# strukturag/libheif

Measured on AMD Instinct MI355X. Metric: Mpixels/s HEIC 4:2:0 8-bit decode, higher is better.
Workload: dtype u8; 1 GPU; 2048 x 3840x2160 HEIC 4:2:0 8-bit stills per GPU and step, WPP, CTB 64, fused YCbCr->RGB24; stage_overlap=False, distinct_contents=256, parallelism=replicas x1

## Files before the change

### libheif_amd/csrc/parse_bins_lds_gfx950.h

```cpp
#define PC_LDS_HEAD_Q   "v_lshrrev_b32 %[vt], 10, %[R]\n\tv_and_b32 %[vt], 24, %[vt]\n\t"
#define PC_LDS_LPS                                                                                                                 \
  "ds_read_b32 %[vn], %[vr] offset:%c[tnext]\n\t"                                                                                   \
  "v_sub_u32 %[val], %[val], %[R]\n\t"                                                                                              \
  "v_ffbh_u32 %[vt], %[vl]\n\t"                                                                                                     \
  "v_add_u32 %[vt], -16, %[vt]\n\t"                                                                                                 \
  "v_lshlrev_b32 %[R], %[vt], %[vl]\n\t"                                                                                            \
  "v_add_u32 %[vt], -7, %[vt]\n\t"                                                                                                  \
  "v_lshlrev_b32 %[val], %[vt], %[val]\n\t"                                                                                         \
  "v_add_u32 %[bits], %[vt], %[bits]\n\t"                                                                                           \
  "v_and_b32 %[vt], 0x10000, %[vst]\n\t"                                                                                            \
  "v_xor_b32 %[vb], 1, %[vb]\n\t"                                                                                                   \
  "s_waitcnt lgkmcnt(0)\n\t"                                                                                                        \
  "v_xor_b32 %[vn], %[vn], %[vt]\n\t"
#if HIPDEC_PARSE_LDS_WIN
#define PC_LDS_REFILL(SLOW)                                                                                                        \
  "s_cmp_lt_u32 %[pos], %[flim]\n\t"                                                                                                \
  "s_cbranch_scc0 " SLOW "\n\t"                                                                                                     \
  "v_lshl_add_u32 %[val], %[vbyte], %[bits], %[val]\n\t"                                                                            \
  "v_add_u32 %[vpos], 1, %[vpos]\n\t"                                                                                               \
  "s_add_u32 %[pos], %[pos], 1\n\t"                                                                                                 \
  "ds_read_u8 %[vbyte], %[vpos] offset:%c[wwin]\n\t"                                                                                \
  "v_add_u32 %[bits], -8, %[bits]\n\t"
#define PC_LDS_WIN_WAIT "s_waitcnt lgkmcnt(0)\n\t"
#define PC_LDS_WIN_STATE(s) [vbyte] "+v"((s).vbyte), [vpos] "+v"((s).vpos),
// ... 26 lines not shown
  PC_LDS_EXP                                                                                                                        \
  "v_and_b32 %[vr], 0xfc, %[vst]\n\t"                                                                                               \
  "ds_read_b32 %[vrow], %[vr] offset:%c[tlps]\n\t"                                                                                  \
  "v_lshrrev_b32 %[vb], 16, %[vst]\n\t"                                                                                             \
  "v_pk_sub_u16 %[vn], %[vst], 4 clamp\n\t"                                                                                         \
  "s_waitcnt lgkmcnt(0)\n\t"                                                                                                        \
  "v_bfe_u32 %[vl], %[vrow], %[vt], 8\n\t"                                                                                          \
  "v_mad_i32_i24 %[R], %[vl], %[m128], %[R]\n\t"                                                                                    \
  "v_cmp_lt_u32_e32 vcc, %[val], %[R]\n\t"                                                                                          \
  "s_cbranch_vccz " LPS_LABEL "\n\t"                                                                                                \
  "v_cmp_gt_u32_e32 vcc, 0x8000, %[R]\n\t"
#define PC_LDS_MPS_SHIFT "v_lshlrev_b32 %[R], 1, %[R]\n\tv_lshlrev_b32 %[val], 1, %[val]\n\tv_add_u32 %[bits], 1, %[bits]\n"
#define PC_LDS_OFFSETS [tlps] "i"(__builtin_offsetof(Lds, tlps)), [tnext] "i"(__builtin_offsetof(Lds, tnext)), [vctx] "i"(__builtin_offsetof(Lds, vctx))
PC_DEV uint32_t pc_lds_ctx_addr(CtxGroup grp, int lane) { return (uint32_t)__builtin_offsetof(Lds, ctx) + 4u * (uint32_t)(grp.base + lane); }

PC_DEV int decode_bin(PS& s, CtxRef grp, int ctx_lane)
{
  uint32_t r, flag;
  [[maybe_unused]] uint32_t st, row;
  uint32_t vst, vrow, vt, vl, vn, vr, vb;
  const uint32_t va = pc_lds_ctx_addr(grp, ctx_lane);
  uint32_t pos = pc_uni(s.pos);
  const uint32_t flim = pc_uni(s.fast_limit);
  asm volatile(
    "ds_read_b32 %[vst], %[va]\n\t"
    "s_mov_b32 %[flag], 0\n\t"
    PC_LDS_HEAD_Q
    "s_waitcnt lgkmcnt(0)\n\t"
    PC_LDS_CORE("1f")
    "s_cbranch_vccz 6f\n\t"
    PC_LDS_MPS_SHIFT
    "s_branch 2f\n"
    "1:\n\t"
    PC_LDS_LPS
    "2:\n\t"
    "v_cmp_lt_i32_e32 vcc, -1, %[bits]\n\t"
// ... 3 lines not shown
    "s_branch 6f\n"
    "3:\n\t"
    "s_mov_b32 %[flag], 1\n"
    "6:\n\t"
    "ds_write_b32 %[va], %[vn]\n\t"
    "v_readfirstlane_b32 %[r], %[vb]\n\t"
    : [R] "+v"(s.range), [val] "+v"(s.value), [bits] "+v"(s.bits_needed), [pos] "+s"(pos), PC_LDS_WIN_STATE(s)
      [r] "=&s"(r), PC_LDS_WIN_TEMPS(st, row) [flag] "=&s"(flag),
      [vst] "=&v"(vst), [vrow] "=&v"(vrow), [vt] "=&v"(vt), [vl] "=&v"(vl), [vn] "=&v"(vn), [vr] "=&v"(vr), [vb] "=&v"(vb)
    : [va] "v"(va), PC_LDS_WIN_IN(s), [flim] "s"(flim), [m128] "v"(0xffffff80u), PC_LDS_OFFSETS
    : "vcc", "scc", "memory");
  s.pos = pc_uni(pos);
  if (__builtin_expect(pc_uni(flag) != 0u, 0)) refill_byte(s);
  return (int)pc_uni(r);
}

#define PC_LDS_SIG_ITER(P, CA, CB, NEXT)                                                                                           \
  "1" P "0:\n\t"                                                                                                                    \
  "ds_read_b32 %[vst], %[" CA "]\n\t"                                                                                               \
  "v_add_u32 %[vj], -4, %[vj]\n\t"                                                                                                  \
  "ds_read_b32 %[" CB "], %[vj] offset:%c[vctx]\n\t"                                                                                \
  PC_LDS_HEAD_Q                                                                                                                     \
  "s_waitcnt lgkmcnt(1)\n\t"                                                                                                        \
  PC_LDS_CORE("1" P "1f")                                                                                                           \
  "s_cbranch_vccnz 1" P "2f\n"                                                                                                      \
  "1" P "4:\n\t"                                                                                                                    \
  "ds_write_b32 %[" CA "], %[vn]\n\t"                                                                                               \
  "v_lshl_or_b32 %[vacc], %[vacc], 1, %[vb]\n\t"                                                                                    \
  "s_add_u32 %[j], %[j], -1\n\t"                                                                                                    \
  "s_cbranch_scc1 " NEXT "\n\t"                                                                                                     \
  "s_branch 190f\n"                                                                                                                 \
  "1" P "1:\n\t"                                                                                                                    \
  PC_LDS_LPS                                                                                                                        \
  "s_branch 1" P "3f\n"                                                                                                             \
  "1" P "2:\n\t"                                                                                                                    \
  PC_LDS_MPS_SHIFT                                                                                                                  \
  "1" P "3:\n\t"                                                                                                                    \
  "v_cmp_lt_i32_e32 vcc, -1, %[bits]\n\t"                                                                                           \
  "s_cbranch_vccz 1" P "4b\n\t"                                                                                                     \
  PC_LDS_REFILL("1" P "5f")                                                                                                         \
  "s_branch 1" P "4b\n"                                                                                                             \
  "1" P "5:\n\t"                                                                                                                    \
  "ds_write_b32 %[" CA "], %[vn]\n\t"                                                                                               \
  "v_lshl_or_b32 %[vacc], %[vacc], 1, %[vb]\n\t"                                                                                    \
  "s_add_u32 %[j], %[j], -1\n\t"                                                                                                    \
  "s_mov_b32 %[flag], 1\n\t"                                                                                                        \
  "s_branch 190f\n"

PC_DEV uint32_t decode_sig_run(PS& s, const VReg& vctx, int n_start)
{
  (void)vctx;
  uint32_t vacc = 0;
  asm volatile("v_mov_b32 %0, 0" : "=v"(vacc));
  int32_t j = __builtin_amdgcn_readfirstlane(n_start - 1);
  for (;;) {
    uint32_t flag, t;
    [[maybe_unused]] uint32_t st, row;
    uint32_t vst, vrow, vt, vl, vn, vr, vb, vca, vcb, vj;
    uint32_t pos = pc_uni(s.pos);
    const uint32_t flim = pc_uni(s.fast_limit);
    asm volatile(
      "s_lshl_b32 %[t], %[j], 2\n\t"
      "s_add_u32 %[t], %[t], 4\n\t"
      "s_mov_b32 %[flag], 0\n\t"
      "v_mov_b32 %[vj], %[t]\n\t"
      "ds_read_b32 %[vca], %[vj] offset:%c[vctx]\n\t"
      "s_waitcnt lgkmcnt(0)\n\t"
      PC_LDS_SIG_ITER("0", "vca", "vcb", "110f")
      PC_LDS_SIG_ITER("1", "vcb", "vca", "100b")
      "190:\n\t"
      PC_LDS_WIN_WAIT
      : [R] "+v"(s.range), [val] "+v"(s.value), [bits] "+v"(s.bits_needed), [pos] "+s"(pos), [j] "+s"(j), [vacc] "+v"(vacc), PC_LDS_WIN_STATE(s)
        [flag] "=&s"(flag), PC_LDS_WIN_TEMPS(st, row) [t] "=&s"(t),
        [vst] "=&v"(vst), [vrow] "=&v"(vrow), [vt] "=&v"(vt), [vl] "=&v"(vl), [vn] "=&v"(vn), [vr] "=&v"(vr), [vb] "=&v"(vb),
        [vca] "=&v"(vca), [vcb] "=&v"(vcb), [vj] "=&v"(vj)
      : PC_LDS_WIN_IN(s), [flim] "s"(flim), [m128] "v"(0xffffff80u), PC_LDS_OFFSETS
      : "vcc", "scc", "memory");
    s.pos = pc_uni(pos);
    if (__builtin_expect(__builtin_amdgcn_readfirstlane((int)flag) != 0, 0)) refill_byte(s);
    j = __builtin_amdgcn_readfirstlane(j);
    if (j < 0) break;
  }
  return pc_uni(vacc) << 1;
}

PC_DEV uint32_t decode_g1_run(PS& s, int base_lane, int n, int& g_io)
{
  uint32_t vgb = 0, vg = 0;
  int32_t m = __builtin_amdgcn_readfirstlane(n - 1);
  const uint32_t vbase = pc_lds_ctx_addr(PS::ctxC, base_lane);
  asm volatile("v_mov_b32 %0, 0\n\tv_mov_b32 %1, %2" : "=&v"(vgb), "=&v"(vg) : "s"((uint32_t)__builtin_amdgcn_readfirstlane(g_io)));
// ... 133 lines not shown
```

### libheif_amd/csrc/parse_core.h

```cpp
#pragma once
#include <stdint.h>
#include "hevc_device.h"

#if defined(HIPDEC_HOST_EMU)
#include <string.h>
#define PC_DEV static inline
inline uint64_t hipdec_emu_path_counts[8] = {};
#define PC_COUNT(k) (hipdec_emu_path_counts[k]++)
inline uint64_t hipdec_emu_glue_counts[32] = {};
#define PC_GLUE(k) (hipdec_emu_glue_counts[k]++)
struct VReg { uint32_t v[64]; };
#define PC_VEC_BEGIN for (int lane = 0; lane < 64; lane++) { (void)lane;
#define PC_VEC_END }
#define PC_L(r) ((r).v[lane])
PC_DEV uint32_t pc_rdlane(const VReg& r, int l) { return r.v[l & 63]; }
PC_DEV void pc_wrlane(VReg& r, int l, uint32_t x) { r.v[l & 63] = x; }
PC_DEV void pc_wrlane_v(VReg& r, int l, uint32_t x) { r.v[l & 63] = x; }
PC_DEV uint32_t pc_uni(uint32_t x) { return x; }
PC_DEV int pc_clz(uint32_t x) { return x ? __builtin_clz(x) : 32; }
PC_DEV int pc_ffs(uint32_t x) { return __builtin_ffs((int)x); }
PC_DEV int pc_popc(uint32_t x) { return __builtin_popcount(x); }
PC_DEV uint64_t pc_ballot(const VReg& r) { uint64_t m = 0; for (int l = 0; l < 64; l++) if (r.v[l]) m |= 1ull << l; return m; }
typedef uint32_t UReg;
PC_DEV UReg pc_vec(uint32_t x) { return x; }
// ... 40 lines not shown
#ifndef HIPDEC_PARSE_CHROMA_GENERAL
#define HIPDEC_PARSE_CHROMA_GENERAL 1
#endif
#ifndef HIPDEC_PARSE_LDS_CTX
#define HIPDEC_PARSE_LDS_CTX 0
#endif
#ifndef HIPDEC_PARSE_LDS_MAPS
#define HIPDEC_PARSE_LDS_MAPS HIPDEC_PARSE_LDS_CTX
#endif
#ifndef HIPDEC_PARSE_LDS_WIN
#define HIPDEC_PARSE_LDS_WIN HIPDEC_PARSE_LDS_CTX
#endif
#ifndef HIPDEC_PARSE_LEAN_GLUE
#define HIPDEC_PARSE_LEAN_GLUE HIPDEC_PARSE_LDS_CTX
#endif
#ifndef HIPDEC_PARSE_INTER
#define HIPDEC_PARSE_INTER 0
#endif

namespace hipdec {
namespace pcore {

struct Lds {
  alignas(16) uint32_t park[SAVE_DWORDS];
#if HIPDEC_PARSE_LDS_CTX
  alignas(16) uint32_t ctx[3 * 64];
  uint32_t tlps[64];
  uint32_t tnext[64];
  uint32_t vctx[16];
#endif
#if HIPDEC_PARSE_LDS_MAPS
  uint32_t umap[5 * 64];
#endif
#if HIPDEC_PARSE_LDS_WIN
  uint32_t wwin[128 + 2];
#endif
};
#if HIPDEC_PARSE_LDS_MAPS
struct UMap { int base; };
typedef UMap MapRef;
#define PC_MAP_SYNC() PC_LDS_SYNC()
#define PC_MAP_DW(s, m) ((s).L->umap[((m).base >> 2) + lane])
#else
typedef VReg& MapRef;
#define PC_MAP_DW(s, m) PC_L(m)
#define PC_MAP_SYNC() do { } while (0)
#endif
#if HIPDEC_PARSE_LDS_CTX
struct CtxGroup { int base; };
typedef CtxGroup CtxRef;
#else
typedef VReg& CtxRef;
// ... 32 lines not shown
  int32_t chroma_format_idc, bit_depth_luma, bit_depth_chroma, log2_min_cu_qp_delta_size;
  uint32_t tools;
  uint32_t pcm;
  int32_t slice_qp_y, deblock, sao_luma, sao_chroma;
  int32_t x_ctb, y_ctb, ctb_avail;
  int32_t is_cu_qp_delta_coded, cu_qp_delta_val, qpy_pred, last_qp_y, cur_qp_y;
  int32_t cu_tq_bypass;
  Lds* L;
#if HIPDEC_PARSE_INTER
  int32_t is_p, num_ref_idx, max_merge_cand, init_type, amp, max_th_depth_inter;
  int32_t is_b, num_ref_idx_l1, mvd_l1_zero;
  MotionSyntax* msyn;
#endif
};
enum : uint32_t { TOOL_SDH = 1, TOOL_TS = 2, TOOL_CUQPD = 4, TOOL_TQBYPASS = 8 };

PC_DEV uint32_t interleave4(uint32_t x, uint32_t y)
{
  x = (x | (x << 2)) & 0x33; x = (x | (x << 1)) & 0x55;
  y = (y | (y << 2)) & 0x33; y = (y | (y << 1)) & 0x55;
  return x | (y << 1);
}
PC_DEV uint32_t compact1by1(uint32_t v)
{
  v &= 0x55555555u; v = (v | (v >> 1)) & 0x33333333u; v = (v | (v >> 2)) & 0x0f0f0f0fu; v = (v | (v >> 4)) & 0x00ff00ffu;
  return v;
}

PC_DEV bool pc_is444(const PS& s) { return HIPDEC_PARSE_CHROMA_GENERAL && s.chroma_format_idc == 3; }
PC_DEV bool pc_is422(const PS& s) { return HIPDEC_PARSE_CHROMA_GENERAL && s.chroma_format_idc == 2; }
// ... 141 lines not shown
{
  s.pos = start; s.end = end; s.zeros = 0; s.win_base = 0xfffff000u; s.fast_limit = 0;
  s.range = pc_vec(510u << 7); s.bits_needed = pc_vec((uint32_t)-8);
  const uint32_t b0 = read_byte(s), b1 = read_byte(s);
  s.value = pc_vec((b0 << 8) | b1);
}
PC_DEV void cabac_restart(PS& s)
{
  s.range = pc_vec(510u << 7); s.bits_needed = pc_vec((uint32_t)-8);
  const uint32_t b0 = read_byte(s), b1 = read_byte(s);
  s.value = pc_vec((b0 << 8) | b1);
}
PC_DEV void refill_byte(PS& s) { s.value += read_byte_v(s) << s.bits_needed; s.bits_needed -= 8u; }

#if HIPDEC_PARSE_LDS_CTX
PC_DEV int decode_bin_cxx(PS& s, CtxRef grp, int ctx_lane)
{
  uint32_t* const cv = &s.L->ctx[grp.base + ctx_lane];
  const uint32_t st = pc_uni(*cv);
  const uint32_t row = pc_uni(s.L->tlps[(st & 0xfcu) >> 2]);
  const UReg lps = (row >> ((s.range >> 10) & 24u)) & 255u;
  UReg range = s.range - (lps << 7);
  uint32_t nst;
  int bin;
  UReg nb;
  if (__builtin_expect(pc_any(s.value < range), 1)) {
    bin = (int)(st >> 16);
    nst = st - (((st & 0xfcu) != 0u) ? 4u : 0u);
    nb = 1u - (range >> 15);
    range <<= nb;
  } else {
    bin = (int)((st >> 16) ^ 1u);
    nb = (UReg)pc_clz(lps) - 23u;
    s.value -= range;
    range = lps << (nb + 7u);
    nst = pc_uni(s.L->tnext[(st & 0xfcu) >> 2]) ^ (st & 0x10000u);
  }
  PC_VEC_BEGIN if (lane == 0) *cv = nst; PC_VEC_END
  s.range = range;
  s.value <<= nb;
  s.bits_needed += nb;
  if (__builtin_expect(pc_any((int32_t)s.bits_needed >= 0), 0)) refill_byte(s);
  return bin;
}
#else
PC_DEV int decode_bin_cxx(PS& s, VReg& grp, int ctx_lane)
{
  const uint32_t st = pc_rdlane(grp, ctx_lane);
  const uint32_t row = pc_rdlane(s.t_lps, (int)st);
  const UReg lps = (row >> ((s.range >> 10) & 24u)) & 255u;
  UReg range = s.range - (lps << 7);
  const UReg vst = pc_vec(st);
  UReg nst;
  int bin;
  UReg nb;
  if (__builtin_expect(pc_any(s.value < range), 1)) {
    bin = (int)(st >> 16);
    nst = vst - (((vst & 63u) != 0u) ? 1u : 0u);
    nb = 1u - (range >> 15);
// ... 31 lines not shown
{
  int i = 0;
  while (i < max && decode_bin(s, grp, base_lane + (i >> shift))) i++;
  return i;
}
PC_DEV uint32_t decode_g1_run(PS& s, int base_lane, int n, int& g)
{
  uint32_t gb = 0;
  for (int i = 0; i < n; i++) {
    const int b = decode_bin(s, s.ctxC, base_lane + (g > 3 ? 3 : g));
    gb = (gb << 1) | (uint32_t)b;
    if (b) g = 0; else if (g > 0) g++;
  }
  return gb;
}
PC_DEV uint32_t decode_sig_run(PS& s, const VReg& vctx, int n_start)
{
  uint32_t sig = 0;
  int k = n_start;
  do sig |= (uint32_t)decode_bin(s, s.ctxB, (int)pc_rdlane(vctx, k)) << k; while (--k > 0);
  return sig;
}
#endif

PC_DEV int decode_bypass(PS& s)
{
  s.value <<= 1;
  s.bits_needed += 1u;
  if (pc_any((int32_t)s.bits_needed >= 0)) { s.bits_needed = pc_vec((uint32_t)-8); s.value += read_byte_v(s); }
  if (pc_any(s.value >= s.range)) { s.value -= s.range; return 1; }
  return 0;
}
PC_DEV uint32_t decode_bypass_multi(PS& s, int n)
{
  s.value <<= n;
  s.bits_needed += (uint32_t)n;
// ... 71 lines not shown
    s.L->tlps[lane] = lps_row;
    s.L->tnext[lane] = (lane < 63 ? (uint32_t)(62 - c_next_lps[ps]) << 2 : 0u) | (lane == 62 ? 0x10000u : 0u);
    PC_L(s.t_next) = (uint32_t)c_diag8[lane] << 8;
#else
    PC_L(s.t_lps) = lps_row;
    PC_L(s.t_next) = (lane < 63 ? (uint32_t)(62 - c_next_lps[ps]) : 0u) | (lane == 62 ? 0x10000u : 0u) | ((uint32_t)c_diag8[lane] << 8);
#endif
  PC_VEC_END
  {
    VReg inv;
    PC_VEC_BEGIN PC_L(inv) = 0u; PC_VEC_END
    for (int k = 0; k < 64; k++) pc_wrlane(inv, (int)((pc_rdlane(s.t_next, k) >> 8) & 63u), (uint32_t)k);
    PC_VEC_BEGIN PC_L(s.t_next) |= PC_L(inv) << 24; PC_VEC_END
  }
}

PC_DEV int left_cb_log2(PS& s, int ux, int uy)
{
  if (ux > 0) return (int)(map_get(s, s.m_size, (int)interleave4((uint32_t)ux - 1, (uint32_t)uy)) >> 4);
  if (s.ctb_avail & AV_LEFT) return (int)((pc_rdlane(s.p_left, uy) & 255u) >> 4);
  return 0;
}
PC_DEV int up_cb_log2(PS& s, int ux, int uy)
{
  if (uy > 0) return (int)(map_get(s, s.m_size, (int)interleave4((uint32_t)ux, (uint32_t)uy - 1)) >> 4);
  if (s.ctb_avail & AV_UP) return (int)(((pc_rdlane(s.up, 9 + (ux >> 2)) >> ((ux & 3) * 8)) & 255u) >> 4);
  return 0;
}
PC_DEV void derive_qp_pred(PS& s, int ux, int uy)
{
// ... 115 lines not shown
  }
  PC_COUNT(2);
  if (!(s.pos < s.fast_limit)) PC_COUNT(3);
  return pc_vec((uint32_t)decode_remaining(s, (int)pc_uni(rice)));
}
PC_DEV void scan_sb(PS& s, int lg, int scan_idx, int i, int& xs, int& ys)
{
  if (lg == 0) { xs = 0; ys = 0; }
  else if (lg == 1) {
    if (scan_idx == 1) { xs = i & 1; ys = i >> 1; }
    else { xs = i >> 1; ys = i & 1; }
  } else if (lg == 2) { const uint32_t v = (uint32_t)(PC_DIAG4 >> (i * 4)) & 15u; xs = (int)(v & 3u); ys = (int)(v >> 2); }
  else { const uint32_t v = (pc_rdlane(s.t_next, i) >> 8) & 63u; xs = (int)(v & 7u); ys = (int)(v >> 3); }
}

PC_DEV int residual_coding(PS& s, int log2n, int c_idx, int pred_mode, int16_t* dst)
{
  const int n = 1 << log2n;
  int ts = 0;
  if ((s.tools & TOOL_TS) && !s.cu_tq_bypass && log2n <= 2) ts = decode_bin(s, s.ctxA, A_TRANSFORM_SKIP + (c_idx ? 1 : 0));
  int ctx_offset, ctx_shift;
  if (c_idx == 0) { ctx_offset = 3 * (log2n - 2) + ((log2n - 1) >> 2); ctx_shift = (log2n + 1) >> 2; }
  else { ctx_offset = 15; ctx_shift = log2n - 2; }
  const int c_max = (log2n << 1) - 1;
  const int px = decode_unary_ctx_run(s, s.ctxA, A_LAST_X + ctx_offset, ctx_shift, c_max);
  const int py = decode_unary_ctx_run(s, s.ctxA, A_LAST_Y + ctx_offset, ctx_shift, c_max);
  int last_x = px, last_y = py;
  if (px > 3) last_x = (1 << ((px >> 1) - 1)) * (2 + (px & 1)) + decode_bypass_bits(s, (px >> 1) - 1);
  if (py > 3) last_y = (1 << ((py >> 1) - 1)) * (2 + (py & 1)) + decode_bypass_bits(s, (py >> 1) - 1);
  int scan_idx = 0;
  if (log2n == 2 || (log2n == 3 && (c_idx == 0 || pc_is444(s)))) {
    if (pred_mode >= 6 && pred_mode <= 14) scan_idx = 2;
    else if (pred_mode >= 22 && pred_mode <= 30) scan_idx = 1;
  }
  if (scan_idx == 2) { const int t = last_x; last_x = last_y; last_y = t; }
  if (last_x >= n || last_y >= n) { s.err = DEV_ERR_SYNTAX; zero_uncoded_sub_blocks(dst, log2n, 0); return ts; }
  const uint64_t scan4 = scan_idx == 0 ? PC_DIAG4 : (scan_idx == 1 ? PC_HORZ4 : PC_VERT4);

  const int lg = log2n - 2;
  int last_sb, last_pos;
  {
    const int xs_t = last_x >> 2, ys_t = last_y >> 2;
    const uint32_t r_t = (uint32_t)((last_x & 3) | ((last_y & 3) << 2));
#if HIPDEC_PARSE_LEAN_GLUE
    last_pos = scan_idx == 0 ? (int)((uint32_t)(PC_INV_DIAG4 >> (r_t * 4u)) & 15u) : (scan_idx == 1 ? (int)r_t : (int)(((r_t & 3u) << 2) | (r_t >> 2)));
#else
    const uint64_t inv4 = scan_idx == 0 ? PC_INV_DIAG4 : (scan_idx == 1 ? PC_INV_HORZ4 : PC_INV_VERT4);
    last_pos = (int)((uint32_t)(inv4 >> (r_t * 4u)) & 15u);
#endif
    if (lg == 0) last_sb = 0;
    else if (lg == 1) last_sb = scan_idx == 1 ? (xs_t | (ys_t << 1)) : ((xs_t << 1) | ys_t);
    else if (lg == 2) last_sb = (int)((uint32_t)(PC_INV_DIAG4 >> ((uint32_t)(xs_t | (ys_t << 2)) * 4u)) & 15u);
    else last_sb = (int)((pc_rdlane(s.t_next, xs_t | (ys_t << 3)) >> 24) & 63u);
  }
  uint64_t csbf = 0;
  const int sbw = 1 << lg;
  (void)sbw;
  if (ts) PC_GLUE(0);
  PC_GLUE(c_idx ? 3 + log2n : log2n - 1);
  if (log2n <= 3) PC_GLUE((log2n == 2 ? 7 : 10) + scan_idx);
  if (lg > 0 && last_sb == 0) PC_GLUE(13);
  if (lg > 0 && last_sb == (1 << (2 * lg)) - 1) PC_GLUE(14);
  if (s.cu_tq_bypass) PC_GLUE(23);
  if (pc_is422(s)) PC_GLUE(27);
  if (pc_is444(s)) PC_GLUE(28);
#if HIPDEC_PARSE_LEAN_GLUE
  int g1_zero = 0;
  const int sdh = (s.tools & TOOL_SDH) != 0 && !s.cu_tq_bypass;
  const int sig_dc = (c_idx == 0 && log2n > 2) ? 3 : 0;
  const int sig_base = log2n == 2 ? (c_idx ? 27 : 0) : (c_idx == 0 ? 3 + (log2n == 3 ? (scan_idx == 0 ? 9 : 15) : 21) : 27 + (log2n == 3 ? 9 : 12));
#else
  int g1_carry = 1, first_sb_with_g1 = 1;
  const int sdh = (s.tools & TOOL_SDH) != 0;
#endif
  VReg vovf;
  PC_VEC_BEGIN PC_L(vovf) = 0u; PC_VEC_END
  for (int i = last_sb; i >= 0; i--) {
    int infer_dc = 0, coded;
#if HIPDEC_PARSE_LEAN_GLUE
    int pos;
    if (lg == 3) pos = (int)((pc_rdlane(s.t_next, i) >> 8) & 63u);
    else if (lg == 2) { const uint32_t v = (uint32_t)(PC_DIAG4 >> (i * 4)) & 15u; pos = (int)((v & 3u) | ((v & 12u) << 1)); }
    else if (lg == 1) pos = scan_idx == 1 ? ((i & 1) | ((i & 2) << 2)) : ((i >> 1) | ((i & 1) << 3));
    else pos = 0;
    const uint32_t nb = (uint32_t)(csbf >> pos) & ((pos & 7) == 7 ? 0x100u : 0x102u);
    if (i < last_sb && i > 0) {
      coded = decode_bin(s, s.ctxA, A_CODED_SUB_BLOCK + (nb ? 1 : 0) + (c_idx ? 2 : 0));
      infer_dc = 1;
      PC_GLUE(coded ? 17 : 16); if (nb & 2u) PC_GLUE(18); if (nb & 0x100u) PC_GLUE(19); if (!nb) PC_GLUE(20);
    } else coded = 1;
    if (!coded) continue;
    const uint32_t pat = log2n == 2 ? 0u : (nb == 0u ? PC_SIGPAT0 : (nb == 2u ? PC_SIGPAT1 : (nb == 0x100u ? PC_SIGPAT2 : PC_SIGPAT3)));
    const int sig_off = sig_base - (pos ? 0 : sig_dc);
    const int xs = pos, ys = 0;
#else
    int xs, ys;
    scan_sb(s, lg, scan_idx, i, xs, ys);
    const int right = (xs < sbw - 1) ? (int)((csbf >> (ys * 8 + xs + 1)) & 1) : 0;
    const int below = (ys < sbw - 1) ? (int)((csbf >> ((ys + 1) * 8 + xs)) & 1) : 0;
    if (i < last_sb && i > 0) {
      coded = decode_bin(s, s.ctxA, A_CODED_SUB_BLOCK + ((right | below) ? 1 : 0) + (c_idx ? 2 : 0));
      infer_dc = 1;
      PC_GLUE(coded ? 17 : 16); if (right) PC_GLUE(18); if (below) PC_GLUE(19); if (!(right | below)) PC_GLUE(20);
    } else coded = 1;
    if (!coded) continue;
    uint32_t pat;
    int sig_off;
    if (log2n == 2) { pat = 0; sig_off = c_idx ? 27 : 0; }
    else {
      const int prev_csbf = right | (below << 1);
      pat = prev_csbf == 0 ? PC_SIGPAT0 : (prev_csbf == 1 ? PC_SIGPAT1 : (prev_csbf == 2 ? PC_SIGPAT2 : PC_SIGPAT3));
      if (c_idx == 0) sig_off = ((xs | ys) ? 3 : 0) + ((log2n == 3) ? (scan_idx == 0 ? 9 : 15) : 21);
      else sig_off = 27 + ((log2n == 3) ? 9 : 12);
    }
#endif
    VReg vctx;
    {
      const int dc_sb = (xs | ys) == 0;
      PC_VEC_BEGIN
        const uint32_t r = (uint32_t)(scan4 >> ((lane & 15) * 4)) & 15u;
        uint32_t c;
        if (log2n == 2) c = (uint32_t)sig_off + (uint32_t)((PC_CTXIDXMAP4 >> (r * 4)) & 15u);
        else if (dc_sb && r == 0) c = c_idx ? 27u : 0u;
        else c = (uint32_t)sig_off + ((pat >> (r * 2)) & 3u);
        PC_L(vctx) = c;
#if HIPDEC_PARSE_LDS_CTX
        if (lane < 16) s.L->vctx[lane] = (uint32_t)__builtin_offsetof(Lds, ctx) + 4u * (uint32_t)(PS::ctxB.base + B_SIG_COEFF) + 4u * c;
#endif
      PC_VEC_END
    }
    uint32_t sig = 0;
    int n_start = 15;
    if (i == last_sb) { sig = 1u << last_pos; n_start = last_pos - 1; }
    if (n_start > 0) {
      sig |= decode_sig_run(s, vctx, n_start);
    }
    if (n_start >= 0) {
      if (infer_dc && !sig) sig = 1u;
      else sig |= (uint32_t)decode_bin(s, s.ctxB, B_SIG_COEFF + (int)pc_rdlane(vctx, 0));
    }
    if (!sig) continue;
#if HIPDEC_PARSE_LEAN_GLUE
    csbf |= 1ull << pos;
#else
    csbf |= 1ull << (ys * 8 + xs);
#endif
#if HIPDEC_PARSE_LEAN_GLUE
    const int ctx_set = ((i == 0 || c_idx > 0) ? 0 : 2) + g1_zero;
#else
    int ctx_set = (i == 0 || c_idx > 0) ? 0 : 2;
    if (!first_sb_with_g1 && g1_carry == 0) ctx_set++;
    first_sb_with_g1 = 0;
#endif
    const int last_sig_pos = 31 - pc_clz(sig), first_sig_pos = pc_ffs(sig) - 1;
// ... 855 lines not shown
  s.is_cu_qp_delta_coded = 0; s.cu_qp_delta_val = 0; s.qpy_pred = s.slice_qp_y; s.last_qp_y = s.slice_qp_y; s.cur_qp_y = s.slice_qp_y;
  s.cu_tq_bypass = 0;

  const int units_log2 = 2 * (s.log2_ctb - 2);
  const int units = 1 << units_log2;
  const int uw = 1 << (s.log2_ctb - 2);
  const int ctb_size = 1 << s.log2_ctb;
  const int n_mincb_log2 = 2 * (s.log2_ctb - s.log2_min_cb);

  load_tables(s);
  PC_VEC_BEGIN
    PC_MAP_DW(s, s.m_size) = 0; PC_MAP_DW(s, s.m_flags) = 0; PC_MAP_DW(s, s.m_ipm) = 0; PC_MAP_DW(s, s.m_ipmc) = 0; PC_MAP_DW(s, s.m_qp) = 0;
    PC_L(s.p_left) = 0; PC_L(s.up) = 0; PC_L(s.sao) = 0; PC_L(s.sao_left) = 0;
#if HIPDEC_PARSE_LDS_CTX
    for (int g = 0; g < 3; g++) s.L->ctx[g * 64 + lane] = 0;
    if (lane < 16) s.L->vctx[lane] = (uint32_t)__builtin_offsetof(Lds, ctx);
#else
    PC_L(s.ctxA) = 0; PC_L(s.ctxB) = 0; PC_L(s.ctxC) = 0;
#endif
    PC_L(s.win) = 0; PC_L(s.win_next) = 0;
  PC_VEC_END
  PC_MAP_SYNC();
  uint32_t k0 = 0;
  uint32_t* saved = A.saved + (size_t)sub_idx * SAVE_DWORDS;
  if (pool) k0 = pc_load_wt_uni(A.resume_k + sub_idx);
  if (k0 == 0) cabac_start(s, byte_start, byte_end);
  else load_row_state(s, saved, 1);

  for (uint32_t k = k0; k < num_ctbs && !s.err; k++) {
    if (pool && A.yield_ctbs && k > k0 && (k - k0) % A.yield_ctbs == 0) {
      save_row_state(s, A.resume_k + sub_idx, saved, k);
// ... 217 lines not shown
    sub = uload32(&A.waves[wave_idx].first); stride = uload32(&A.waves[wave_idx].stride);
    end = uload32(&A.waves[wave_idx].end); lag = uload32(&A.waves[wave_idx].start_lag);
  } else {
    const uint32_t n_init = A.num_waves < 64u ? A.num_waves : 64u;
    for (uint32_t s0 = wave_idx; wave_idx < n_init && s0 < A.num_subs; s0 += n_init) {
      const int32_t dep = (int32_t)uload32(&A.subs[s0].dep_sub);
      if (dep < 0) pool_push(A, s0);
      else {
        uint32_t need = 2u;
        const uint32_t dep_len = uload32(&A.subs[s0].dep_len);
        if (need > dep_len || (uload32(&A.subs[s0].wpp_sync) & 255u) == 2u) need = dep_len;
        if (pool_arm(A, s0, (uint32_t)dep, need)) pool_push(A, s0);
      }
    }
  }
#if defined(HIPDEC_POOL_TRACE) && !defined(HIPDEC_HOST_EMU)
  unsigned long long tr_start = 0, tr_last = 0, tr_idle = 0, tr_tasks = 0, tr_busy = 0, tr_now0 = wall_clock64();
#endif
  for (;;) {
    uint32_t* slot = A.queue;
#if defined(HIPDEC_POOL_TRACE) && !defined(HIPDEC_HOST_EMU)
    tr_now0 = wall_clock64();
#endif
    if (!pool) { if (sub >= end) return; }
    else {
#if defined(HIPDEC_POOL_TRACE) && !defined(HIPDEC_HOST_EMU)
      const unsigned long long tr_now = wall_clock64();
      if (tr_tasks == 0 && tr_idle == 0) tr_start = tr_now;
      if (threadIdx.x == 0 && A.trace) {
        unsigned long long* tr = A.trace + (size_t)wave_idx * 32;
// ... 48 lines not shown
```

### libheif_amd/csrc/parse_tables.h

```cpp
#pragma once
#include <stdint.h>
#ifndef PC_CONST
#define PC_CONST static const
#endif

namespace hipdec {
namespace pcore {

enum : int {
  A_SAO_MERGE = 0, A_SAO_TYPE = 1, A_SPLIT_CU = 2 , A_CU_TQ_BYPASS = 5, A_PART_MODE = 6, A_PREV_INTRA_LUMA = 7,
  A_INTRA_CHROMA = 8, A_SPLIT_TRANSFORM = 9 , A_CBF_LUMA = 12 , A_CBF_CHROMA = 14 , A_CU_QP_DELTA = 18 ,
  A_TRANSFORM_SKIP = 20 , A_LAST_X = 22 , A_LAST_Y = 40 , A_CODED_SUB_BLOCK = 58 ,
  A_CBF_CHROMA4 = 62 ,
  B_SIG_COEFF = 0, B_GREATER2 = 44,
  C_GREATER1 = 0,
  C_SKIP_FLAG = 24 , C_PRED_MODE = 27, C_PART_MODE_INTER = 28 , C_MERGE_FLAG = 31,
  C_MERGE_IDX = 32, C_REF_IDX = 33 , C_MVD_GT0 = 35, C_MVD_GT1 = 36, C_MVP_FLAG = 37, C_RQT_ROOT_CBF = 38,
  C_INTER_PRED_IDC = 39
};

PC_CONST uint8_t c_init[3][64] = {
  {153, 200, 139, 141, 157, 154, 184, 184, 63, 153, 138, 138, 111, 141, 94, 138, 182, 154, 154, 154, 139, 139,
   110, 110, 124, 125, 140, 153, 125, 127, 140, 109, 111, 143, 127, 111, 79, 108, 123, 63,
   110, 110, 124, 125, 140, 153, 125, 127, 140, 109, 111, 143, 127, 111, 79, 108, 123, 63,
// ... 71 lines not shown
  uint32_t w = 0;
  for (int r = 0; r < 16; r++) {
    const int x = r & 3, y = r >> 2;
    int v = 2;
    if (prev_csbf == 0) v = (x + y == 0) ? 2 : (x + y < 3) ? 1 : 0;
    else if (prev_csbf == 1) v = (y == 0) ? 2 : (y == 1) ? 1 : 0;
    else if (prev_csbf == 2) v = (x == 0) ? 2 : (x == 1) ? 1 : 0;
    else v = 2;
    w |= (uint32_t)v << (2 * r);
  }
  return w;
}
constexpr uint32_t PC_SIGPAT0 = pc_sigpat(0), PC_SIGPAT1 = pc_sigpat(1), PC_SIGPAT2 = pc_sigpat(2), PC_SIGPAT3 = pc_sigpat(3);
static_assert(PC_SIGPAT0 == 0x00010516u && PC_SIGPAT1 == 0x000055AAu && PC_SIGPAT2 == 0x06060606u && PC_SIGPAT3 == 0xAAAAAAAAu, "sig patterns");

}
}
```

Baseline: 19940 Mpixel/s.

## Precompute sig_coeff context-address rows and TU descriptors in LDS tables

Builds compile-time tables of per-position sig_coeff_flag context LDS addresses, grouped by TU size, component, scan and neighbour pattern, plus a per-TU-kind descriptor holding ctx offsets, scan words and sub-block scan offsets. These tables are copied into LDS at kernel start. The residual-coding sig run now reads 16-bit context addresses straight from a table row, replacing the per-sub-block vector computation of vctx and its LDS write. The aim is to cut scalar/vector glue and syncs in the hot CABAC residual path, at the cost of extra LDS footprint, a startup copy, and more complex address bookkeeping.

```diff
diff --git a/libheif_amd/csrc/parse_bins_lds_gfx950.h b/libheif_amd/csrc/parse_bins_lds_gfx950.h
--- a/libheif_amd/csrc/parse_bins_lds_gfx950.h
+++ b/libheif_amd/csrc/parse_bins_lds_gfx950.h
@@ -64,12 +64,11 @@
 #define PC_LDS_OFFSETS [tlps] "i"(__builtin_offsetof(Lds, tlps)), [tnext] "i"(__builtin_offsetof(Lds, tnext)), [vctx] "i"(__builtin_offsetof(Lds, vctx))
 PC_DEV uint32_t pc_lds_ctx_addr(CtxGroup grp, int lane) { return (uint32_t)__builtin_offsetof(Lds, ctx) + 4u * (uint32_t)(grp.base + lane); }
 
-PC_DEV int decode_bin(PS& s, CtxRef grp, int ctx_lane)
+PC_DEV int decode_bin_at(PS& s, uint32_t va)
 {
   uint32_t r, flag;
   [[maybe_unused]] uint32_t st, row;
   uint32_t vst, vrow, vt, vl, vn, vr, vb;
-  const uint32_t va = pc_lds_ctx_addr(grp, ctx_lane);
   uint32_t pos = pc_uni(s.pos);
   const uint32_t flim = pc_uni(s.fast_limit);
   asm volatile(
@@ -103,12 +102,19 @@
   if (__builtin_expect(pc_uni(flag) != 0u, 0)) refill_byte(s);
   return (int)pc_uni(r);
 }
-
+PC_DEV int decode_bin(PS& s, CtxRef grp, int ctx_lane) { return decode_bin_at(s, pc_lds_ctx_addr(grp, ctx_lane)); }
+
+#if HIPDEC_PARSE_TU_TABLES
+#define PC_LDS_SIG_ROW_IN [srow] "s"(srow),
+#define PC_LDS_SIG_NEXT(CB) "v_add_u32 %[vj], -2, %[vj]\n\tds_read_u16 %[" CB "], %[vj]\n\t"
+#else
+#define PC_LDS_SIG_ROW_IN
+#define PC_LDS_SIG_NEXT(CB) "v_add_u32 %[vj], -4, %[vj]\n\tds_read_b32 %[" CB "], %[vj] offset:%c[vctx]\n\t"
+#endif
 #define PC_LDS_SIG_ITER(P, CA, CB, NEXT)                                                                                           \
   "1" P "0:\n\t"                                                                                                                    \
   "ds_read_b32 %[vst], %[" CA "]\n\t"                                                                                               \
-  "v_add_u32 %[vj], -4, %[vj]\n\t"                                                                                                  \
-  "ds_read_b32 %[" CB "], %[vj] offset:%c[vctx]\n\t"                                                                                \
+  PC_LDS_SIG_NEXT(CB)                                                                                                               \
   PC_LDS_HEAD_Q                                                                                                                     \
   "s_waitcnt lgkmcnt(1)\n\t"                                                                                                        \
   PC_LDS_CORE("1" P "1f")                                                                                                           \
@@ -136,9 +142,15 @@
   "s_mov_b32 %[flag], 1\n\t"                                                                                                        \
   "s_branch 190f\n"
 
+#if HIPDEC_PARSE_TU_TABLES
+PC_DEV uint32_t decode_sig_run_row(PS& s, uint32_t row_addr, int n_start)
+{
+  const uint32_t srow = pc_uni(row_addr);
+#else
 PC_DEV uint32_t decode_sig_run(PS& s, const VReg& vctx, int n_start)
 {
   (void)vctx;
+#endif
   uint32_t vacc = 0;
   asm volatile("v_mov_b32 %0, 0" : "=v"(vacc));
   int32_t j = __builtin_amdgcn_readfirstlane(n_start - 1);
@@ -149,11 +161,18 @@
     uint32_t pos = pc_uni(s.pos);
     const uint32_t flim = pc_uni(s.fast_limit);
     asm volatile(
+#if HIPDEC_PARSE_TU_TABLES
+      "s_lshl1_add_u32 %[t], %[j], %[srow]\n\t"
+      "s_mov_b32 %[flag], 0\n\t"
+      "v_add_u32_e64 %[vj], %[t], 2\n\t"
+      "ds_read_u16 %[vca], %[vj]\n\t"
+#else
       "s_lshl_b32 %[t], %[j], 2\n\t"
       "s_add_u32 %[t], %[t], 4\n\t"
       "s_mov_b32 %[flag], 0\n\t"
       "v_mov_b32 %[vj], %[t]\n\t"
       "ds_read_b32 %[vca], %[vj] offset:%c[vctx]\n\t"
+#endif
       "s_waitcnt lgkmcnt(0)\n\t"
       PC_LDS_SIG_ITER("0", "vca", "vcb", "110f")
       PC_LDS_SIG_ITER("1", "vcb", "vca", "100b")
@@ -163,7 +182,7 @@
         [flag] "=&s"(flag), PC_LDS_WIN_TEMPS(st, row) [t] "=&s"(t),
         [vst] "=&v"(vst), [vrow] "=&v"(vrow), [vt] "=&v"(vt), [vl] "=&v"(vl), [vn] "=&v"(vn), [vr] "=&v"(vr), [vb] "=&v"(vb),
         [vca] "=&v"(vca), [vcb] "=&v"(vcb), [vj] "=&v"(vj)
-      : PC_LDS_WIN_IN(s), [flim] "s"(flim), [m128] "v"(0xffffff80u), PC_LDS_OFFSETS
+      : PC_LDS_SIG_ROW_IN PC_LDS_WIN_IN(s), [flim] "s"(flim), [m128] "v"(0xffffff80u), PC_LDS_OFFSETS
       : "vcc", "scc", "memory");
     s.pos = pc_uni(pos);
     if (__builtin_expect(__builtin_amdgcn_readfirstlane((int)flag) != 0, 0)) refill_byte(s);
diff --git a/libheif_amd/csrc/parse_core.h b/libheif_amd/csrc/parse_core.h
--- a/libheif_amd/csrc/parse_core.h
+++ b/libheif_amd/csrc/parse_core.h
@@ -78,6 +78,18 @@
 #ifndef HIPDEC_PARSE_LEAN_GLUE
 #define HIPDEC_PARSE_LEAN_GLUE HIPDEC_PARSE_LDS_CTX
 #endif
+#ifndef HIPDEC_PARSE_TU_TABLES
+#define HIPDEC_PARSE_TU_TABLES HIPDEC_PARSE_LDS_CTX
+#endif
+#if HIPDEC_PARSE_TU_TABLES && !(HIPDEC_PARSE_LDS_CTX && HIPDEC_PARSE_LEAN_GLUE)
+#error "HIPDEC_PARSE_TU_TABLES: the sig-context rows live in LDS beside the context variables, and the row arithmetic is the lean glue's"
+#endif
+#ifndef HIPDEC_PARSE_TU_DESC
+#define HIPDEC_PARSE_TU_DESC HIPDEC_PARSE_TU_TABLES
+#endif
+#if HIPDEC_PARSE_TU_DESC && !HIPDEC_PARSE_TU_TABLES
+#error "HIPDEC_PARSE_TU_DESC: the descriptor holds addresses of the sig-context rows"
+#endif
 #ifndef HIPDEC_PARSE_INTER
 #define HIPDEC_PARSE_INTER 0
 #endif
@@ -85,6 +97,7 @@
 namespace hipdec {
 namespace pcore {
 
+#define PC_SIG_ROWS (HIPDEC_PARSE_CHROMA_GENERAL ? PC_SIG_ROWS_ALL : PC_SIG_ROWS_420)
 struct Lds {
   alignas(16) uint32_t park[SAVE_DWORDS];
 #if HIPDEC_PARSE_LDS_CTX
@@ -99,7 +112,26 @@
 #if HIPDEC_PARSE_LDS_WIN
   uint32_t wwin[128 + 2];
 #endif
+#if HIPDEC_PARSE_TU_TABLES
+  uint16_t sigrow[PC_SIG_ROWS * 16];
+#endif
+#if HIPDEC_PARSE_TU_DESC
+  uint8_t sbscan[PC_SBSCAN_BYTES];
+#endif
 };
+#if HIPDEC_PARSE_LDS_CTX
+#define PC_LDS_CTX_B_ADDR ((uint32_t)__builtin_offsetof(Lds, ctx) + 4u * (64u + (uint32_t)B_SIG_COEFF))
+#endif
+#if HIPDEC_PARSE_TU_TABLES
+static_assert(pc_sig_rows_match(PC_LDS_CTX_B_ADDR), "sig_coeff_flag context rows against 9.3.4.2.5 as residual_coding derived it");
+static_assert(__builtin_offsetof(Lds, sigrow) % 4 == 0 && sizeof(Lds) < 65536, "sig rows are copied by dwords and hold 16-bit LDS addresses");
+PC_CONST SigRowTable c_sig_rows = pc_make_sig_rows(PC_LDS_CTX_B_ADDR);
+#endif
+#if HIPDEC_PARSE_TU_DESC
+static_assert(sizeof(Lds) < (1u << 13) && __builtin_offsetof(Lds, sbscan) % 4 == 0, "the descriptor holds 13-bit LDS addresses; the scans are copied by dwords");
+PC_CONST TuDescTable c_tu_desc = pc_make_tu_desc((uint32_t)__builtin_offsetof(Lds, sigrow));
+PC_CONST SbScanTable c_sbscan = pc_make_sbscan();
+#endif
 #if HIPDEC_PARSE_LDS_MAPS
 struct UMap { int base; };
 typedef UMap MapRef;
@@ -162,6 +194,14 @@
 #endif
 };
 enum : uint32_t { TOOL_SDH = 1, TOOL_TS = 2, TOOL_CUQPD = 4, TOOL_TQBYPASS = 8 };
+#if HIPDEC_PARSE_LDS_CTX
+static_assert(PS::ctxB.base == 64, "PC_LDS_CTX_B_ADDR");
+#endif
+#if HIPDEC_PARSE_TU_TABLES
+PC_DEV UReg pc_lds_u16(PS& s, uint32_t addr) { return *(const uint16_t*)((const uint8_t*)s.L + addr); }
+PC_DEV UReg pc_lds_u8(PS& s, uint32_t addr) { return *((const uint8_t*)s.L + addr); }
+PC_DEV uint32_t tu_sig_row(uint32_t rows, uint32_t rows_dc, uint32_t nb, int pos) { return (pos ? rows : rows_dc) + (((nb << 4) | (nb >> 2)) & 96u); }
+#endif
 
 PC_DEV uint32_t interleave4(uint32_t x, uint32_t y)
 {
@@ -333,9 +373,9 @@
 PC_DEV void refill_byte(PS& s) { s.value += read_byte_v(s) << s.bits_needed; s.bits_needed -= 8u; }
 
 #if HIPDEC_PARSE_LDS_CTX
-PC_DEV int decode_bin_cxx(PS& s, CtxRef grp, int ctx_lane)
-{
-  uint32_t* const cv = &s.L->ctx[grp.base + ctx_lane];
+PC_DEV int decode_bin_cxx_at(PS& s, uint32_t ctx_addr)
+{
+  uint32_t* const cv = (uint32_t*)((uint8_t*)s.L + ctx_addr);
   const uint32_t st = pc_uni(*cv);
   const uint32_t row = pc_uni(s.L->tlps[(st & 0xfcu) >> 2]);
   const UReg lps = (row >> ((s.range >> 10) & 24u)) & 255u;
@@ -362,6 +402,7 @@
   if (__builtin_expect(pc_any((int32_t)s.bits_needed >= 0), 0)) refill_byte(s);
   return bin;
 }
+PC_DEV int decode_bin_cxx(PS& s, CtxRef grp, int ctx_lane) { return decode_bin_cxx_at(s, (uint32_t)__builtin_offsetof(Lds, ctx) + 4u * (uint32_t)(grp.base + ctx_lane)); }
 #else
 PC_DEV int decode_bin_cxx(PS& s, VReg& grp, int ctx_lane)
 {
@@ -423,12 +464,34 @@
   }
   return gb;
 }
+#if HIPDEC_PARSE_LDS_CTX
+PC_DEV int decode_bin_at(PS& s, UReg ctx_addr) { return decode_bin_cxx_at(s, pc_uni(ctx_addr)); }
+#endif
+#if HIPDEC_PARSE_TU_TABLES
+PC_DEV uint32_t decode_sig_run_row(PS& s, uint32_t row, int n_start)
+{
+  uint32_t sig = 0;
+  int k = n_start;
+  do sig |= (uint32_t)decode_bin_at(s, pc_uni(*(const uint16_t*)((const uint8_t*)s.L + row + 2u * (uint32_t)k))) << k; while (--k > 0);
+  return sig;
+}
+#else
 PC_DEV uint32_t decode_sig_run(PS& s, const VReg& vctx, int n_start)
 {
   uint32_t sig = 0;
   int k = n_start;
   do sig |= (uint32_t)decode_bin(s, s.ctxB, (int)pc_rdlane(vctx, k)) << k; while (--k > 0);
   return sig;
+}
+#endif
+#endif
+#if HIPDEC_PARSE_TU_TABLES
+PC_DEV uint32_t decode_sig_run(PS& s, const VReg& vctx, int n_start)
+{
+  PC_LDS_SYNC();
+  PC_VEC_BEGIN if (lane < 16) ((uint16_t*)s.L->vctx)[lane] = (uint16_t)(PC_LDS_CTX_B_ADDR + 4u * PC_L(vctx)); PC_VEC_END
+  PC_LDS_SYNC();
+  return decode_sig_run_row(s, (uint32_t)__builtin_offsetof(Lds, vctx), n_start);
 }
 #endif
 
@@ -530,6 +593,21 @@
     PC_VEC_BEGIN PC_L(s.t_next) |= PC_L(inv) << 24; PC_VEC_END
   }
 }
+
+#if HIPDEC_PARSE_TU_TABLES
+PC_DEV void load_tu_tables(Lds* L)
+{
+  const uint32_t* const src = (const uint32_t*)c_sig_rows.a;
+  uint32_t* const dst = (uint32_t*)L->sigrow;
+  PC_VEC_BEGIN
+    for (int k = lane; k < PC_SIG_ROWS * 8; k += 64) dst[k] = src[k];
+#if HIPDEC_PARSE_TU_DESC
+    if (lane < PC_SBSCAN_BYTES / 4) ((uint32_t*)L->sbscan)[lane] = ((const uint32_t*)c_sbscan.a)[lane];
+#endif
+  PC_VEC_END
+  PC_LDS_SYNC();
+}
+#endif
 
 PC_DEV int left_cb_log2(PS& s, int ux, int uy)
 {
@@ -675,28 +753,55 @@
   else { const uint32_t v = (pc_rdlane(s.t_next, i) >> 8) & 63u; xs = (int)(v & 7u); ys = (int)(v >> 3); }
 }
 
+PC_DEV int tu_scan_idx(PS& s, int log2n, int c_idx, int pred_mode)
+{
+  int scan_idx = 0;
+  if (log2n == 2 || (log2n == 3 && (c_idx == 0 || pc_is444(s)))) {
+    if (pred_mode >= 6 && pred_mode <= 14) scan_idx = 2;
+    else if (pred_mode >= 22 && pred_mode <= 30) scan_idx = 1;
+  }
+  return scan_idx;
+}
 PC_DEV int residual_coding(PS& s, int log2n, int c_idx, int pred_mode, int16_t* dst)
 {
   const int n = 1 << log2n;
   int ts = 0;
+#if HIPDEC_PARSE_TU_DESC
+  const int scan_idx_d = tu_scan_idx(s, log2n, c_idx, pred_mode);
+  typedef uint32_t u32x4 __attribute__((vector_size(16)));
+  const u32x4 desc = *(const u32x4*)c_tu_desc.w[(uint32_t)pc_tu_kind(log2n, c_idx, scan_idx_d)];
+  const uint32_t d0 = desc[0], d1 = desc[1], d2 = desc[2], d3 = desc[3];
+#endif
   if ((s.tools & TOOL_TS) && !s.cu_tq_bypass && log2n <= 2) ts = decode_bin(s, s.ctxA, A_TRANSFORM_SKIP + (c_idx ? 1 : 0));
+#if HIPDEC_PARSE_TU_DESC
+  const int ctx_offset = (int)(d1 & 31u), ctx_shift = (int)((d1 >> 5) & 3u), c_max = (int)((d1 >> 7) & 15u);
+#else
   int ctx_offset, ctx_shift;
   if (c_idx == 0) { ctx_offset = 3 * (log2n - 2) + ((log2n - 1) >> 2); ctx_shift = (log2n + 1) >> 2; }
   else { ctx_offset = 15; ctx_shift = log2n - 2; }
   const int c_max = (log2n << 1) - 1;
+#endif
   const int px = decode_unary_ctx_run(s, s.ctxA, A_LAST_X + ctx_offset, ctx_shift, c_max);
   const int py = decode_unary_ctx_run(s, s.ctxA, A_LAST_Y + ctx_offset, ctx_shift, c_max);
   int last_x = px, last_y = py;
   if (px > 3) last_x = (1 << ((px >> 1) - 1)) * (2 + (px & 1)) + decode_bypass_bits(s, (px >> 1) - 1);
   if (py > 3) last_y = (1 << ((py >> 1) - 1)) * (2 + (py & 1)) + decode_bypass_bits(s, (py >> 1) - 1);
+#if HIPDEC_PARSE_TU_DESC
+  const int scan_idx = scan_idx_d;
+#else
   int scan_idx = 0;
   if (log2n == 2 || (log2n == 3 && (c_idx == 0 || pc_is444(s)))) {
     if (pred_mode >= 6 && pred_mode <= 14) scan_idx = 2;
     else if (pred_mode >= 22 && pred_mode <= 30) scan_idx = 1;
   }
+#endif
   if (scan_idx == 2) { const int t = last_x; last_x = last_y; last_y = t; }
   if (last_x >= n || last_y >= n) { s.err = DEV_ERR_SYNTAX; zero_uncoded_sub_blocks(dst, log2n, 0); return ts; }
+#if HIPDEC_PARSE_TU_DESC
+  const uint64_t scan4 = (uint64_t)d2 | ((uint64_t)d3 << 32);
+#else
   const uint64_t scan4 = scan_idx == 0 ? PC_DIAG4 : (scan_idx == 1 ? PC_HORZ4 : PC_VERT4);
+#endif
 
   const int lg = log2n - 2;
   int last_sb, last_pos;
@@ -719,6 +824,7 @@
   (void)sbw;
   if (ts) PC_GLUE(0);
   PC_GLUE(c_idx ? 3 + log2n : log2n - 1);
+  if (c_idx && log2n == 4) PC_GLUE(15);
   if (log2n <= 3) PC_GLUE((log2n == 2 ? 7 : 10) + scan_idx);
   if (lg > 0 && last_sb == 0) PC_GLUE(13);
   if (lg > 0 && last_sb == (1 << (2 * lg)) - 1) PC_GLUE(14);
@@ -728,8 +834,21 @@
 #if HIPDEC_PARSE_LEAN_GLUE
   int g1_zero = 0;
   const int sdh = (s.tools & TOOL_SDH) != 0 && !s.cu_tq_bypass;
+#if HIPDEC_PARSE_TU_TABLES
+#if HIPDEC_PARSE_TU_DESC
+  const uint32_t sig_rows = d0 & 0xffffu, sig_rows_dc = d0 >> 16, sig_dc0 = d1 >> 18;
+  const uint32_t sb_scan = (uint32_t)__builtin_offsetof(Lds, sbscan) + ((d1 >> 11) & 127u);
+#else
+  const uint32_t sig_rows = (uint32_t)__builtin_offsetof(Lds, sigrow) + (uint32_t)PC_SIG_ROW_BYTES *
+      (uint32_t)(log2n == 2 ? (c_idx ? 3 : 0) + scan_idx
+                            : (c_idx == 0 ? (log2n == 3 ? 6 + 8 * scan_idx : 30) : (log2n == 3 ? ((HIPDEC_PARSE_CHROMA_GENERAL && scan_idx) ? 42 + 4 * scan_idx : 38) : 42)));
+  const uint32_t sig_rows_dc = sig_rows + ((c_idx == 0 && log2n > 2) ? (uint32_t)PC_SIG_DC_STEP : 0u);
+  const uint32_t sig_dc0 = (uint32_t)__builtin_offsetof(Lds, sigrow) + (c_idx ? 3u * PC_SIG_ROW_BYTES : 0u);
+#endif
+#else
   const int sig_dc = (c_idx == 0 && log2n > 2) ? 3 : 0;
   const int sig_base = log2n == 2 ? (c_idx ? 27 : 0) : (c_idx == 0 ? 3 + (log2n == 3 ? (scan_idx == 0 ? 9 : 15) : 21) : 27 + (log2n == 3 ? 9 : 12));
+#endif
 #else
   int g1_carry = 1, first_sb_with_g1 = 1;
   const int sdh = (s.tools & TOOL_SDH) != 0;
@@ -740,10 +859,14 @@
     int infer_dc = 0, coded;
 #if HIPDEC_PARSE_LEAN_GLUE
     int pos;
+#if HIPDEC_PARSE_TU_DESC
+    pos = (int)pc_uni(pc_lds_u8(s, sb_scan + (uint32_t)i));
+#else
     if (lg == 3) pos = (int)((pc_rdlane(s.t_next, i) >> 8) & 63u);
     else if (lg == 2) { const uint32_t v = (uint32_t)(PC_DIAG4 >> (i * 4)) & 15u; pos = (int)((v & 3u) | ((v & 12u) << 1)); }
     else if (lg == 1) pos = scan_idx == 1 ? ((i & 1) | ((i & 2) << 2)) : ((i >> 1) | ((i & 1) << 3));
     else pos = 0;
+#endif
     const uint32_t nb = (uint32_t)(csbf >> pos) & ((pos & 7) == 7 ? 0x100u : 0x102u);
     if (i < last_sb && i > 0) {
       coded = decode_bin(s, s.ctxA, A_CODED_SUB_BLOCK + (nb ? 1 : 0) + (c_idx ? 2 : 0));
@@ -751,9 +874,14 @@
       PC_GLUE(coded ? 17 : 16); if (nb & 2u) PC_GLUE(18); if (nb & 0x100u) PC_GLUE(19); if (!nb) PC_GLUE(20);
     } else coded = 1;
     if (!coded) continue;
+#if HIPDEC_PARSE_TU_TABLES
+    const uint32_t sig_row = tu_sig_row(sig_rows, sig_rows_dc, nb, pos);
+    const UReg va0 = pc_lds_u16(s, pos ? sig_row : sig_dc0);
+#else
     const uint32_t pat = log2n == 2 ? 0u : (nb == 0u ? PC_SIGPAT0 : (nb == 2u ? PC_SIGPAT1 : (nb == 0x100u ? PC_SIGPAT2 : PC_SIGPAT3)));
     const int sig_off = sig_base - (pos ? 0 : sig_dc);
     const int xs = pos, ys = 0;
+#endif
 #else
     int xs, ys;
     scan_sb(s, lg, scan_idx, i, xs, ys);
@@ -775,6 +903,7 @@
       else sig_off = 27 + ((log2n == 3) ? 9 : 12);
     }
 #endif
+#if !HIPDEC_PARSE_TU_TABLES
     VReg vctx;
     {
       const int dc_sb = (xs | ys) == 0;
@@ -790,15 +919,24 @@
 #endif
       PC_VEC_END
     }
+#endif
     uint32_t sig = 0;
     int n_start = 15;
     if (i == last_sb) { sig = 1u << last_pos; n_start = last_pos - 1; }
     if (n_start > 0) {
+#if HIPDEC_PARSE_TU_TABLES
+      sig |= decode_sig_run_row(s, sig_row, n_start);
+#else
       sig |= decode_sig_run(s, vctx, n_start);
+#endif
     }
     if (n_start >= 0) {
       if (infer_dc && !sig) sig = 1u;
+#if HIPDEC_PARSE_TU_TABLES
+      else sig |= (uint32_t)decode_bin_at(s, va0);
+#else
       else sig |= (uint32_t)decode_bin(s, s.ctxB, B_SIG_COEFF + (int)pc_rdlane(vctx, 0));
+#endif
     }
     if (!sig) continue;
 #if HIPDEC_PARSE_LEAN_GLUE
@@ -1684,7 +1822,9 @@
     PC_L(s.p_left) = 0; PC_L(s.up) = 0; PC_L(s.sao) = 0; PC_L(s.sao_left) = 0;
 #if HIPDEC_PARSE_LDS_CTX
     for (int g = 0; g < 3; g++) s.L->ctx[g * 64 + lane] = 0;
+#if !HIPDEC_PARSE_TU_TABLES
     if (lane < 16) s.L->vctx[lane] = (uint32_t)__builtin_offsetof(Lds, ctx);
+#endif
 #else
     PC_L(s.ctxA) = 0; PC_L(s.ctxB) = 0; PC_L(s.ctxC) = 0;
 #endif
@@ -1932,6 +2072,9 @@
       }
     }
   }
+#if HIPDEC_PARSE_TU_TABLES
+  load_tu_tables(lds);
+#endif
 #if defined(HIPDEC_POOL_TRACE) && !defined(HIPDEC_HOST_EMU)
   unsigned long long tr_start = 0, tr_last = 0, tr_idle = 0, tr_tasks = 0, tr_busy = 0, tr_now0 = wall_clock64();
 #endif
diff --git a/libheif_amd/csrc/parse_tables.h b/libheif_amd/csrc/parse_tables.h
--- a/libheif_amd/csrc/parse_tables.h
+++ b/libheif_amd/csrc/parse_tables.h
@@ -109,5 +109,105 @@
 constexpr uint32_t PC_SIGPAT0 = pc_sigpat(0), PC_SIGPAT1 = pc_sigpat(1), PC_SIGPAT2 = pc_sigpat(2), PC_SIGPAT3 = pc_sigpat(3);
 static_assert(PC_SIGPAT0 == 0x00010516u && PC_SIGPAT1 == 0x000055AAu && PC_SIGPAT2 == 0x06060606u && PC_SIGPAT3 == 0xAAAAAAAAu, "sig patterns");
 
-}
-}
+constexpr uint32_t pc_sig_ctx(int log2n, int c_idx, int scan_idx, int right, int below, int dc_sb, int k)
+{
+  const uint64_t scan4 = scan_idx == 0 ? PC_DIAG4 : (scan_idx == 1 ? PC_HORZ4 : PC_VERT4);
+  const uint32_t r = (uint32_t)(scan4 >> (k * 4)) & 15u;
+  if (log2n == 2) return (c_idx ? 27u : 0u) + (uint32_t)((PC_CTXIDXMAP4 >> (r * 4)) & 15u);
+  if (dc_sb && r == 0) return c_idx ? 27u : 0u;
+  const uint32_t pat = pc_sigpat(right | (below << 1));
+  const uint32_t off = c_idx == 0 ? (dc_sb ? 0u : 3u) + (log2n == 3 ? (scan_idx == 0 ? 9u : 15u) : 21u) : 27u + (log2n == 3 ? 9u : 12u);
+  return off + ((pat >> (r * 2)) & 3u);
+}
+enum : int { PC_SIG_ROWS_420 = 46, PC_SIG_ROWS_ALL = 54, PC_SIG_ROW_BYTES = 32, PC_SIG_DC_STEP = 4 * PC_SIG_ROW_BYTES };
+constexpr int pc_sig_row_group(int log2n, int c_idx, int scan_idx)
+{
+  if (log2n == 2) return (c_idx ? 3 : 0) + scan_idx;
+  if (c_idx == 0) return log2n == 3 ? 6 + 8 * scan_idx : 30;
+  return log2n == 3 ? (scan_idx == 0 ? 38 : 46 + 4 * (scan_idx - 1)) : 42;
+}
+constexpr int pc_sig_dc_step(int log2n, int c_idx) { return (c_idx == 0 && log2n > 2) ? PC_SIG_DC_STEP : 0; }
+struct alignas(4) SigRowTable { uint16_t a[PC_SIG_ROWS_ALL * 16]; };
+constexpr SigRowTable pc_make_sig_rows(uint32_t ctx_b_addr)
+{
+  SigRowTable t = {};
+  for (int c_idx = 0; c_idx < 2; c_idx++)
+    for (int log2n = 2; log2n <= 5; log2n++)
+      for (int scan_idx = 0; scan_idx < (log2n <= 3 ? 3 : 1); scan_idx++)
+        for (int nbp = 0; nbp < (log2n == 2 ? 1 : 4); nbp++)
+          for (int dc = 0; dc < 2; dc++) {
+            if (dc && pc_sig_dc_step(log2n, c_idx) == 0 && log2n > 2) continue;
+            if (log2n == 2 && !dc) continue;
+            const int row = pc_sig_row_group(log2n, c_idx, scan_idx) + nbp + (dc && log2n > 2 ? PC_SIG_DC_STEP / PC_SIG_ROW_BYTES : 0);
+            for (int k = 0; k < 16; k++) t.a[row * 16 + k] = (uint16_t)(ctx_b_addr + 4u * pc_sig_ctx(log2n, c_idx, scan_idx, nbp & 1, nbp >> 1, dc, k));
+          }
+  return t;
+}
+constexpr bool pc_sig_rows_match(uint32_t ctx_b_addr)
+{
+  const SigRowTable t = pc_make_sig_rows(ctx_b_addr);
+  for (int c_idx = 0; c_idx < 2; c_idx++)
+    for (int log2n = 2; log2n <= 5; log2n++)
+      for (int scan_idx = 0; scan_idx < (log2n <= 3 ? 3 : 1); scan_idx++)
+        for (int nbp = 0; nbp < (log2n == 2 ? 1 : 4); nbp++)
+          for (int dc = (log2n == 2 ? 1 : 0); dc < 2; dc++) {
+            const int row_bytes = pc_sig_row_group(log2n, c_idx, scan_idx) * PC_SIG_ROW_BYTES + (nbp & 1) * 32 + (nbp >> 1) * 64 + (dc ? pc_sig_dc_step(log2n, c_idx) : 0);
+            if (row_bytes % PC_SIG_ROW_BYTES || row_bytes / PC_SIG_ROW_BYTES >= PC_SIG_ROWS_ALL) return false;
+            if (!(c_idx && log2n == 3 && scan_idx) && row_bytes / PC_SIG_ROW_BYTES >= PC_SIG_ROWS_420) return false;
+            for (int k = 0; k < 16; k++) {
+              const int at = (k == 0 && dc) ? pc_sig_row_group(2, c_idx, 0) * 16 : row_bytes / 2 + k;
+              if (t.a[at] != ctx_b_addr + 4u * pc_sig_ctx(log2n, c_idx, scan_idx, nbp & 1, nbp >> 1, dc, k)) return false;
+            }
+          }
+  return true;
+}
+
+
+enum : int { PC_TU_KINDS = 24 };
+constexpr int pc_tu_kind(int log2n, int c_idx, int scan_idx) { return ((c_idx ? 4 : 0) + log2n - 2) * 3 + scan_idx; }
+struct DiagScan { uint8_t a[64]; };
+constexpr DiagScan pc_diag_scan(int n, int shift)
+{
+  DiagScan d = {};
+  int i = 0, x = 0, y = 0;
+  for (;;) {
+    while (y >= 0) { if (x < n && y < n) d.a[i++] = (uint8_t)(x | (y << shift)); y--; x++; }
+    y = x; x = 0;
+    if (i >= n * n) break;
+  }
+  return d;
+}
+static_assert(pc_diag_scan(4, 2).a[3] == ((PC_DIAG4 >> 12) & 15u) && pc_diag_scan(4, 2).a[9] == ((PC_DIAG4 >> 36) & 15u) && pc_diag_scan(4, 2).a[15] == 15, "6.5.3 against PC_DIAG4");
+enum : int { PC_SBSCAN_1 = 0, PC_SBSCAN_2D = 4, PC_SBSCAN_2H = 8, PC_SBSCAN_4 = 12, PC_SBSCAN_8 = 28, PC_SBSCAN_BYTES = 92 };
+struct alignas(4) SbScanTable { uint8_t a[PC_SBSCAN_BYTES]; };
+constexpr SbScanTable pc_make_sbscan()
+{
+  SbScanTable t = {};
+  for (int i = 0; i < 4; i++) { t.a[PC_SBSCAN_2D + i] = (uint8_t)((i >> 1) | ((i & 1) << 3)); t.a[PC_SBSCAN_2H + i] = (uint8_t)((i & 1) | ((i >> 1) << 3)); }
+  for (int i = 0; i < 16; i++) t.a[PC_SBSCAN_4 + i] = pc_diag_scan(4, 3).a[i];
+  for (int i = 0; i < 64; i++) t.a[PC_SBSCAN_8 + i] = pc_diag_scan(8, 3).a[i];
+  return t;
+}
+constexpr int pc_sbscan_of(int log2n, int scan_idx) { return log2n == 2 ? PC_SBSCAN_1 : (log2n == 3 ? (scan_idx == 1 ? PC_SBSCAN_2H : PC_SBSCAN_2D) : (log2n == 4 ? PC_SBSCAN_4 : PC_SBSCAN_8)); }
+struct alignas(16) TuDescTable { uint32_t w[PC_TU_KINDS][4]; };
+constexpr TuDescTable pc_make_tu_desc(uint32_t sigrow_addr)
+{
+  TuDescTable t = {};
+  for (int c_idx = 0; c_idx < 2; c_idx++)
+    for (int log2n = 2; log2n <= 5; log2n++)
+      for (int scan_idx = 0; scan_idx < (log2n <= 3 ? 3 : 1); scan_idx++) {
+        uint32_t* const w = t.w[pc_tu_kind(log2n, c_idx, scan_idx)];
+        const uint32_t rows = sigrow_addr + (uint32_t)(pc_sig_row_group(log2n, c_idx, scan_idx) * PC_SIG_ROW_BYTES);
+        w[0] = rows | ((rows + (uint32_t)pc_sig_dc_step(log2n, c_idx)) << 16);
+        const uint32_t ctx_offset = c_idx == 0 ? (uint32_t)(3 * (log2n - 2) + ((log2n - 1) >> 2)) : 15u;
+        const uint32_t ctx_shift = c_idx == 0 ? (uint32_t)((log2n + 1) >> 2) : (uint32_t)(log2n - 2);
+        const uint32_t dc0 = sigrow_addr + (uint32_t)(pc_sig_row_group(2, c_idx, 0) * PC_SIG_ROW_BYTES);
+        w[1] = ctx_offset | (ctx_shift << 5) | ((uint32_t)(2 * log2n - 1) << 7) | ((uint32_t)pc_sbscan_of(log2n, scan_idx) << 11) | (dc0 << 18);
+        const uint64_t scan4 = scan_idx == 0 ? PC_DIAG4 : (scan_idx == 1 ? PC_HORZ4 : PC_VERT4);
+        w[2] = (uint32_t)scan4; w[3] = (uint32_t)(scan4 >> 32);
+      }
+  return t;
+}
+
+}
+}
```

Measured after the change: 20680 Mpixel/s (median of 6 runs). 1.04x the previous value.
